# thu-ml/zhusuan

Measured on NVIDIA H100. Metric: leapfrog-steps*chains/sec, higher is better.
Workload: dtype f32

## Files before the change

zhusuan_b200/csrc/hmc_dense_res.cu:

```cuda
#include "hmc_dense_epilogue.cuh"

namespace {

struct ResEpi {
  const __half* __restrict__ hi_cur; const __half* __restrict__ lo_cur;
  __half* __restrict__ hi_nxt; __half* __restrict__ lo_nxt;
  const __half* __restrict__ hi_cur_s; const __half* __restrict__ lo_cur_s;
  __half* __restrict__ hi_nxt_s; __half* __restrict__ lo_nxt_s;
  const float* __restrict__ p_in; float* __restrict__ p_out;
  float* __restrict__ lp_part; float* __restrict__ k_part;
  int64_t chains; int D;
  float sq, inv_sq, acc_scale;
  float rescale;
};

template <int MODE, int NEXT, int DC, bool SPARE>
__device__ __forceinline__ void epilogue_planes(const ResEpi& a, uint32_t trow, int n, bool n_ok,
                                                int64_t c0, int64_t part_row, int lane, float s2,
                                                float eps_over_m_sq, float inv_m, float b_n,
                                                float mu_n, float& qmax) {
  constexpr int NCOL = BN;
  const uint32_t D = DC ? (uint32_t)DC : (uint32_t)a.D;
  const int64_t chains = a.chains;
  const bool warp_n_ok = __all_sync(0xffffffffu, n_ok);
  const bool fast_tile = warp_n_ok && (c0 + NCOL <= chains);
  const int64_t off_t = c0 * (int64_t)D + n;
  const float* __restrict__ pin0 = a.p_in + off_t;
  float* __restrict__ po0 = a.p_out + off_t;
  const unsigned short* __restrict__ hc0 =
      reinterpret_cast<const unsigned short*>(a.hi_cur) + off_t;
  const unsigned short* __restrict__ lc0 =
      reinterpret_cast<const unsigned short*>(a.lo_cur) + off_t;
  __half* __restrict__ hn0 = NEXT ? a.hi_nxt + off_t : nullptr;
  __half* __restrict__ ln0 = NEXT ? a.lo_nxt + off_t : nullptr;
  __half* __restrict__ hs0 = SPARE ? a.hi_nxt_s + off_t : nullptr;
  __half* __restrict__ ls0 = SPARE ? a.lo_nxt_s + off_t : nullptr;

  auto element = [&](float acc, float p, uint32_t hl, float& pn, float& lpv, float& kv,
                     float& Qn) {
    const float Q = __half2float(__ushort_as_half((unsigned short)(hl & 0xFFFFu))) +
                    __half2float(__ushort_as_half((unsigned short)(hl >> 16)));
    const float g = b_n - a.acc_scale * acc;
    pn = fmaf(s2, g, p);
    if (MODE >= 1) lpv = (Q * a.inv_sq - mu_n) * g;
    if (MODE >= 2) kv = pn * pn * inv_m;
    if (NEXT) Qn = fmaf(eps_over_m_sq, pn, Q);
  };

  if (fast_tile) {
    auto load = [&](float* pe, uint32_t* he, int c) {
      const size_t cb = (size_t)c * D;
#pragma unroll
      for (int j = 0; j < 16; ++j) {
        pe[j] = __ldcg(pin0 + cb + (uint32_t)j * D);
        const uint32_t h = __ldcg(hc0 + cb + (uint32_t)j * D);
        const uint32_t l = __ldcg(lc0 + cb + (uint32_t)j * D);
        he[j] = h | (l << 16);
      }
    };
    float ss_a = 0.f, ss_b = 0.f;
    auto compute = [&](const uint32_t* v, const float* pe, const uint32_t* he, int c, float& ss) {
      const size_t cb = (size_t)c * D;
      float lpv[MODE >= 1 ? 16 : 1], kv[MODE >= 2 ? 16 : 1];
#pragma unroll
      for (int j = 0; j < 16; j += 2) {
        float pn[2], lp1[2] = {0.f, 0.f}, k1[2] = {0.f, 0.f}, Qn[2] = {0.f, 0.f};
#pragma unroll
        for (int t = 0; t < 2; ++t) {
          element(__uint_as_float(v[j + t]), pe[j + t], he[j + t], pn[t], lp1[t], k1[t], Qn[t]);
          po0[cb + (uint32_t)(j + t) * D] = pn[t];
          if (MODE >= 1) lpv[j + t] = lp1[t];
          if (MODE >= 2) kv[j + t] = k1[t];
          if (NEXT && !SPARE) ss = fmaf(Qn[t], Qn[t], ss);
          if (SPARE) qmax = fmaxf(qmax, fabsf(Qn[t]));
        }
        if (NEXT) {
          const __half2 h2 = __floats2half2_rn(Qn[0], Qn[1]);
          const float2 hf = __half22float2(h2);
          const __half2 l2 = __floats2half2_rn(Qn[0] - hf.x, Qn[1] - hf.y);
          hn0[cb + (uint32_t)j * D] = __low2half(h2);
          hn0[cb + (uint32_t)(j + 1) * D] = __high2half(h2);
          ln0[cb + (uint32_t)j * D] = __low2half(l2);
          ln0[cb + (uint32_t)(j + 1) * D] = __high2half(l2);
        }
        if (SPARE) {
          const float x0 = Qn[0] * a.rescale, x1 = Qn[1] * a.rescale;
          const __half2 h2 = __floats2half2_rn(x0, x1);
          const float2 hf = __half22float2(h2);
          const __half2 l2 = __floats2half2_rn(x0 - hf.x, x1 - hf.y);
          hs0[cb + (uint32_t)j * D] = __low2half(h2);
          hs0[cb + (uint32_t)(j + 1) * D] = __high2half(h2);
          ls0[cb + (uint32_t)j * D] = __low2half(l2);
          ls0[cb + (uint32_t)(j + 1) * D] = __high2half(l2);
        }
      }
      if (MODE >= 1) {
        const float sum = warp_transpose_sum16(lpv, lane);
        if (lane < 16) a.lp_part[part_row + c0 + c + lane] = sum;
      }
      if (MODE >= 2) {
        const float sum = warp_transpose_sum16(kv, lane);
        if (lane < 16) a.k_part[part_row + c0 + c + lane] = sum;
      }
    };
    float pa[16], pb[16];
    uint32_t ha[16], hb[16], va[16], vb[16];
    load(pa, ha, 0);
#pragma unroll 1
    for (int c = 0; c < NCOL; c += 32) {
      load(pb, hb, c + 16);
      acc_ld16(trow + 4u * (uint32_t)c, va);
      compute(va, pa, ha, c, ss_a);
      if (c + 32 < NCOL) load(pa, ha, c + 32);
      acc_ld16(trow + 4u * (uint32_t)(c + 16), vb);
      compute(vb, pb, hb, c + 16, ss_b);
    }
    if (NEXT && !SPARE) {
      const float norm = sqrtf(ss_a + ss_b) * (1.f + 0x1p-10f);
      qmax = fmaxf(qmax, norm == norm ? norm : INFINITY);
    }
  } else {
#pragma unroll 1
    for (int c = 0; c < NCOL; c += 16) {
      uint32_t v[16];
      acc_ld16(trow + 4u * (uint32_t)c, v);
      const int64_t cbase = c0 + c;
      if (cbase < chains) {
        const size_t cb = (size_t)c * D;
        float lpv[MODE >= 1 ? 16 : 1], kv[MODE >= 2 ? 16 : 1];
#pragma unroll
        for (int j = 0; j < 16; ++j) {
          const bool ok = n_ok && cbase + j < chains;
          float p = 0.f;
          uint32_t hl = 0u;
          if (ok) {
            p = __ldcg(pin0 + cb + (uint32_t)j * D);
            hl = (uint32_t)__ldcg(hc0 + cb + (uint32_t)j * D) |
                 ((uint32_t)__ldcg(lc0 + cb + (uint32_t)j * D) << 16);
          }
          float pn, lp1 = 0.f, k1 = 0.f, Qn = 0.f;
          element(__uint_as_float(v[j]), p, hl, pn, lp1, k1, Qn);
          const __half hh = __float2half_rn(Qn);
          const __half ll = __float2half_rn(Qn - __half2float(hh));
          if (NEXT && ok) qmax = fmaxf(qmax, fabsf(Qn));
          if (MODE >= 1) lpv[j] = ok ? lp1 : 0.f;
          if (MODE >= 2) kv[j] = ok ? k1 : 0.f;
          if (ok) {
            po0[cb + (uint32_t)j * D] = pn;
            if (NEXT) {
              hn0[cb + (uint32_t)j * D] = hh;
              ln0[cb + (uint32_t)j * D] = ll;
            }
            if (SPARE) {
              const float x = Qn * a.rescale;
              const __half hs = __float2half_rn(x);
              hs0[cb + (uint32_t)j * D] = hs;
              ls0[cb + (uint32_t)j * D] = __float2half_rn(x - __half2float(hs));
            }
          }
        }
        if (MODE >= 1) {
          const float sum = warp_transpose_sum16(lpv, lane);
          if (lane < 16 && cbase + lane < chains) a.lp_part[part_row + cbase + lane] = sum;
        }
        if (MODE >= 2) {
          const float sum = warp_transpose_sum16(kv, lane);
          if (lane < 16 && cbase + lane < chains) a.k_part[part_row + cbase + lane] = sum;
        }
      }
    }
  }
}


__device__ __forceinline__ int& producer_spare_in() {
  __shared__ int spare_in;
  return spare_in;
}

template <int MODE, int NEXT, int DC, int CX, int CY>
struct ResW {
  static constexpr int KIND = 1, RB = 64, MNA = 0, MNB = 0;
  static constexpr int CLUSTER = CX * CY;
  static constexpr int KE = RB / 2;
  static constexpr uint32_t TX = Cfg<RB>::STAGE;
  CUtensorMap m_phi, m_plo, m_qhi, m_qlo, m_shi, m_slo;
  ResEpi ea;
  const float* bvec; const float* mu; const float* mass; const float* state;
  float* scales;
  float p_scale;
  int n_blk, D_rt, pass;
  struct EpiState { float qmax = 0.f; };

  __device__ __forceinline__ int D() const { return DC ? DC : D_rt; }
  __host__ __device__ __forceinline__ int64_t units() const {
    return ((ea.chains + BN - 1) / BN) * (int64_t)n_blk;
  }
  __device__ __forceinline__ void tile(int64_t u, int& nb, int64_t& cb) const {
    const uint64_t cu = (uint64_t)u / CLUSTER;
    const int r = (int)((uint64_t)u % CLUSTER);
    const uint32_t nbx = (uint32_t)(n_blk / CX);
    nb = (int)(cu % nbx) * CX + r % CX;
    cb = (int64_t)(cu / nbx) * CY + r / CX;
  }
  __device__ __forceinline__ void kb_range(int64_t, int& kb0, int& kb1) const {
    kb0 = 0;
    kb1 = D() / KE;
  }
  __device__ __forceinline__ void prefetch() const {
    tma_prefetch_desc(&m_phi); tma_prefetch_desc(&m_plo);
    tma_prefetch_desc(&m_qhi); tma_prefetch_desc(&m_qlo);
    tma_prefetch_desc(&m_shi); tma_prefetch_desc(&m_slo);
    producer_spare_in() = plane_spare_in(scales, pass);
  }
  __device__ __forceinline__ void load(int64_t u, int kb, uint32_t sa, uint32_t fb) const {
    using C = Cfg<RB>;
    int nb;
    int64_t cb;
    tile(u, nb, cb);
    const int n0 = nb * BM;
    const int c0 = (int)cb * BN;
    const bool s = producer_spare_in() != 0;
    const CUtensorMap* qh = s ? &m_shi : &m_qhi;
    const CUtensorMap* ql = s ? &m_slo : &m_qlo;
    const int r = (int)(u % CLUSTER), rx = r % CX, ry = r / CX;
    if constexpr (CY == 1) {
      tma_load_2d(sa, &m_phi, fb, kb * KE, n0);
      tma_load_2d(sa + C::A_TILE, &m_plo, fb, kb * KE, n0);
    } else {
      constexpr int rows = BM / CY;
      uint16_t mask = 0;
#pragma unroll
      for (int y = 0; y < CY; ++y) mask |= (uint16_t)(1u << (y * CX + rx));
      const uint32_t o = (uint32_t)(ry * rows * RB);
      tma_load_2d_mc(sa + o, &m_phi, fb, kb * KE, n0 + ry * rows, mask);
      tma_load_2d_mc(sa + C::A_TILE + o, &m_plo, fb, kb * KE, n0 + ry * rows, mask);
    }
    if constexpr (CX == 1) {
      tma_load_2d(sa + 2 * C::A_TILE, qh, fb, kb * KE, c0);
      tma_load_2d(sa + 2 * C::A_TILE + C::B_TILE, ql, fb, kb * KE, c0);
    } else {
      constexpr int rows = BN / CX;
      const uint16_t mask = (uint16_t)(((1u << CX) - 1u) << (ry * CX));
      const uint32_t o = (uint32_t)(rx * rows * RB);
      tma_load_2d_mc(sa + 2 * C::A_TILE + o, qh, fb, kb * KE, c0 + rx * rows, mask);
      tma_load_2d_mc(sa + 2 * C::A_TILE + C::B_TILE + o, ql, fb, kb * KE, c0 + rx * rows, mask);
    }
  }
  __device__ __forceinline__ float sq_alt(float eps, float sq) const {
    return next_plane_scale(scales, pass, eps, mul(eps, p_scale), sq);
  }
  __device__ __forceinline__ void epilogue(int64_t u, uint32_t trow, int quarter, int lane,
                                           EpiState& st) const {
    int nb;
    int64_t cb;
    tile(u, nb, cb);
    const int n = nb * BM + quarter * 32 + lane;
    const int64_t c0 = cb * BN;
    const bool n_ok = n < D();
    const float eps = state[ZSB_ST_EPS_USED];
    const float s2 = mul(eps, p_scale);
    const bool spare_in = plane_spare_in(scales, pass);
    const float sq = plane_scale_in(scales, pass);
    const float m_n = n_ok ? mass[n] : 1.f;
    const float eps_over_m_sq = mul(fdiv(eps, m_n), sq);
    const float inv_m = fdiv(1.f, m_n);
    const float b_n = (n_ok && bvec) ? bvec[n] : 0.f;
    const float mu_n = (n_ok && mu) ? mu[n] : 0.f;
    const int64_t part_row = (int64_t)(nb * 4 + quarter) * ea.chains;
    ResEpi a = ea;
    if (spare_in) {
      a.hi_cur = ea.hi_cur_s;
      a.lo_cur = ea.lo_cur_s;
    }
    a.sq = sq;
    a.inv_sq = fdiv(1.f, sq);
    a.acc_scale = 1.f / (scales[3] * sq);
    a.rescale = NEXT ? sq_alt(eps, sq) * a.inv_sq : 1.f;
    if (a.rescale == 1.f)
      epilogue_planes<MODE, NEXT, DC, false>(a, trow, n, n_ok, c0, part_row, lane, s2,
                                             eps_over_m_sq, inv_m, b_n, mu_n, st.qmax);
    else
      epilogue_planes<MODE, NEXT, DC, true>(a, trow, n, n_ok, c0, part_row, lane, s2,
                                            eps_over_m_sq, inv_m, b_n, mu_n, st.qmax);
  }
  __device__ __forceinline__ void epi_finish(EpiState& st, int quarter, int lane) const {
    if (!NEXT) return;
    const float sq = plane_scale_in(scales, pass);
    const float alt = sq_alt(state[ZSB_ST_EPS_USED], sq);
    publish_plane_scale(scales, pass, sq, alt, st.qmax * (1.f / sq),
                        alt != sq && !(st.qmax < kHalfOverflow), quarter, lane);
  }
};

constexpr int RES_CX = 2, RES_CY = 1;

template <int DC, int CX, int CY>
int res_pass(const CUtensorMap& phi, const CUtensorMap& plo, const CUtensorMap& qhi,
             const CUtensorMap& qlo, const CUtensorMap& shi, const CUtensorMap& slo,
             const ResEpi& ea, const float* bvec, const float* mu, const float* mass,
             const float* state, float* scales, int pass, float p_scale, int n_blk, int D,
             int mode, cudaStream_t st) {
  if (mode == 1) {
    const ResW<1, 1, DC, CX, CY> w{phi, plo, qhi, qlo, shi, slo, ea, bvec, mu, mass, state,
                                   scales, p_scale, n_blk, D, pass};
    return tc_launch(w, st, "hmc_dense_resident");
  }
  if (mode == 0) {
    const ResW<0, 1, DC, CX, CY> w{phi, plo, qhi, qlo, shi, slo, ea, bvec, mu, mass, state,
                                   scales, p_scale, n_blk, D, pass};
    return tc_launch(w, st, "hmc_dense_resident");
  }
  const ResW<2, 0, DC, CX, CY> w{phi, plo, qhi, qlo, shi, slo, ea, bvec, mu, mass, state, scales,
                                 p_scale, n_blk, D, pass};
  return tc_launch(w, st, "hmc_dense_resident");
}

template <int DC>
int res_pass(bool cluster, const CUtensorMap& phi, const CUtensorMap& plo, const CUtensorMap& qhi,
             const CUtensorMap& qlo, const CUtensorMap& shi, const CUtensorMap& slo,
             const ResEpi& ea, const float* bvec, const float* mu, const float* mass,
             const float* state, float* scales, int pass, float p_scale, int n_blk, int D,
             int mode, cudaStream_t st) {
  return cluster ? res_pass<DC, RES_CX, RES_CY>(phi, plo, qhi, qlo, shi, slo, ea, bvec, mu, mass,
                                                state, scales, pass, p_scale, n_blk, D, mode, st)
                 : res_pass<DC, 1, 1>(phi, plo, qhi, qlo, shi, slo, ea, bvec, mu, mass, state,
                                      scales, pass, p_scale, n_blk, D, mode, st);
}

__global__ void __launch_bounds__(256) select_planes_kernel(float* __restrict__ q,
                                                            const __half* __restrict__ planes,
                                                            const __half* __restrict__ spare,
                                                            const float* __restrict__ record,
                                                            const int32_t* __restrict__ accept,
                                                            int64_t chains, int64_t D) {
  const bool use_spare = __float_as_uint(record[3]) != 0u;
  const float inv_sq = 1.f / record[use_spare ? 1 : 0];
  if (use_spare) planes = spare;
  const int lane = threadIdx.x & 31;
  const int n8 = (int)(D >> 3);
  const int64_t wstride = (int64_t)gridDim.x * 8;
  for (int64_t c = (int64_t)blockIdx.x * 8 + (threadIdx.x >> 5); c < chains; c += wstride) {
    if (!accept[c]) continue;
    const uint4* __restrict__ hi = reinterpret_cast<const uint4*>(planes + c * D);
    const uint4* __restrict__ lo = reinterpret_cast<const uint4*>(planes + (chains + c) * D);
    float4* __restrict__ qr = reinterpret_cast<float4*>(q + c * D);
    for (int i0 = lane; i0 < n8; i0 += 128) {
      uint4 h[4], l[4];
#pragma unroll
      for (int u = 0; u < 4; ++u) {
        const int i = i0 + 32 * u;
        if (i < n8) { h[u] = __ldcs(hi + i); l[u] = __ldcs(lo + i); }
      }
#pragma unroll
      for (int u = 0; u < 4; ++u) {
        const int i = i0 + 32 * u;
        if (i < n8) {
          const uint32_t hw[4] = {h[u].x, h[u].y, h[u].z, h[u].w};
          const uint32_t lw[4] = {l[u].x, l[u].y, l[u].z, l[u].w};
          float o[8];
#pragma unroll
          for (int k = 0; k < 4; ++k) {
            const float2 hf = __half22float2(*reinterpret_cast<const __half2*>(&hw[k]));
            const float2 lf = __half22float2(*reinterpret_cast<const __half2*>(&lw[k]));
            o[2 * k] = (hf.x + lf.x) * inv_sq;
            o[2 * k + 1] = (hf.y + lf.y) * inv_sq;
          }
          qr[2 * i] = make_float4(o[0], o[1], o[2], o[3]);
          qr[2 * i + 1] = make_float4(o[4], o[5], o[6], o[7]);
        }
      }
    }
  }
}

}

int zsb_dense_res_h16_launch(void* planes0, void* planes1, void* spare0, void* spare1,
                             const float* p0, float* pw,
                             const void* P_h16, const void* P_l16, float* scales,
                             const float* bvec, const float* mu, const float* mass,
                             const float* state, float* lp0_part, float* lp1_part, float* k_part,
                             int64_t chains, int D, int L, cudaStream_t st) {
  if (D % 64 != 0 || D < 64 || L < 1 || chains <= 0 || chains >= (1LL << 31)) {
    zsb_set_error("dense_res: needs D %% 64 == 0, n_leapfrogs >= 1");
    return ZSB_ERR_INVALID;
  }
  if (planes0 == planes1 || !spare0 || !spare1 || spare0 == spare1) {
    zsb_set_error("dense_res: planes1, spare0 and spare1 must be separate work buffers");
    return ZSB_ERR_INVALID;
  }
  const int n_blk = (D + BM - 1) / BM;
  const int64_t c_blk = (chains + BN - 1) / BN;
  const bool cluster = n_blk % RES_CX == 0 && c_blk % RES_CY == 0;
  const uint32_t p_box = cluster ? BM / RES_CY : BM, q_box = cluster ? BN / RES_CX : BN;
  CUtensorMap phi, plo, qhi[2], qlo[2], shi[2], slo[2];
  int rc;
  constexpr int RB = ResW<0, 1, 0, 1, 1>::RB;
  if ((rc = make_map(&phi, P_h16, (uint64_t)D, (uint64_t)D, p_box, RB, 1))) return rc;
  if ((rc = make_map(&plo, P_l16, (uint64_t)D, (uint64_t)D, p_box, RB, 1))) return rc;
  __half* pl[2] = {reinterpret_cast<__half*>(planes0), reinterpret_cast<__half*>(planes1)};
  __half* sp[2] = {reinterpret_cast<__half*>(spare0), reinterpret_cast<__half*>(spare1)};
  const int64_t plane = chains * (int64_t)D;
  for (int b = 0; b < 2; ++b) {
    if ((rc = make_map(&qhi[b], pl[b], (uint64_t)chains, (uint64_t)D, q_box, RB, 1))) return rc;
    if ((rc = make_map(&qlo[b], pl[b] + plane, (uint64_t)chains, (uint64_t)D, q_box, RB, 1)))
      return rc;
    if ((rc = make_map(&shi[b], sp[b], (uint64_t)chains, (uint64_t)D, q_box, RB, 1))) return rc;
    if ((rc = make_map(&slo[b], sp[b] + plane, (uint64_t)chains, (uint64_t)D, q_box, RB, 1)))
      return rc;
  }
  for (int i = 0; i <= L; ++i) {
    const bool last = i == L;
    const int buf = i & 1;
    const ResEpi ea{pl[buf], pl[buf] + plane, pl[buf ^ 1], pl[buf ^ 1] + plane,
                    sp[buf], sp[buf] + plane, sp[buf ^ 1], sp[buf ^ 1] + plane,
                    i == 0 ? p0 : pw, pw, i == 0 ? lp0_part : lp1_part, k_part, chains, D,
                    1.f, 1.f, 1.f, 1.f};
    const int mode = last ? 2 : (i == 0 ? 1 : 0);
    const float p_scale = (i > 0 && !last) ? 1.f : 0.5f;
    rc = (D == 1024)
             ? res_pass<1024>(cluster, phi, plo, qhi[buf], qlo[buf], shi[buf], slo[buf], ea, bvec,
                              mu, mass, state, scales, i, p_scale, n_blk, D, mode, st)
             : res_pass<0>(cluster, phi, plo, qhi[buf], qlo[buf], shi[buf], slo[buf], ea, bvec, mu,
                           mass, state, scales, i, p_scale, n_blk, D, mode, st);
    if (rc != ZSB_OK) return rc;
  }
  return ZSB_OK;
}

#ifdef ZSB_PASS_PROFILE
extern "C" int zsb_pass_profile_read(unsigned long long* host, int ctas) {
  if (ctas < 0 || ctas > PASS_PROF_CTAS) return ZSB_ERR_INVALID;
  const size_t bytes = sizeof(unsigned long long) * PASS_PROF_SLOTS * (size_t)ctas;
  if (cudaMemcpyFromSymbol(host, g_pass_prof, bytes) != cudaSuccess) return ZSB_ERR_CUDA;
  static unsigned long long zeros[PASS_PROF_CTAS * PASS_PROF_SLOTS];
  if (cudaMemcpyToSymbol(g_pass_prof, zeros, sizeof(zeros)) != cudaSuccess) return ZSB_ERR_CUDA;
  return ZSB_OK;
}
#endif

int zsb_dense_select_planes_launch(float* q, const void* planes, const void* spare,
                                   const float* record, const int32_t* accept, int64_t chains,
                                   int64_t D, cudaStream_t st) {
  ZSB_REQUIRE(D % 8 == 0, "zsb_dense_select_planes: D must be a multiple of 8");
  int64_t blocks = zsb_ceil_div(chains, 8);
  if (blocks > ZSB_NUM_SMS * 16) blocks = ZSB_NUM_SMS * 16;
  if (blocks < 1) blocks = 1;
  select_planes_kernel<<<(unsigned)blocks, 256, 0, st>>>(
      q, reinterpret_cast<const __half*>(planes), reinterpret_cast<const __half*>(spare), record,
      accept, chains, D);
  return zsb_check_launch("hmc_select_planes");
}
```

zhusuan_b200/csrc/tc_common.cuh:

```cuda
#pragma once
#include "common.cuh"
#include <cuda.h>
#include <cuda_fp16.h>

namespace {

constexpr int BM = 128;
constexpr int BN = 128;
constexpr int NUM_EPI_WARPS = 4;
constexpr int PRODUCER_WARP = 4;
constexpr int EPI_WARP0 = 5;
constexpr int NUM_THREADS = 32 * (EPI_WARP0 + NUM_EPI_WARPS);
constexpr int ACC_LD = BN + 4;
constexpr int ACC_BYTES = BM * ACC_LD * 4;
constexpr unsigned long long WAIT_TIMEOUT_NS = 2000000000ULL;

enum PassProfSlot {
  PROF_MMA_TOTAL,
  PROF_MMA_FULL,
  PROF_MMA_TEMPTY,
  PROF_MMA_STORE,
  PROF_PROD_EMPTY,
  PROF_EPI_TFULL,
  PROF_EPI_UNIT,
  PROF_UNITS,
  PASS_PROF_SLOTS
};
constexpr int PASS_PROF_CTAS = 1024;
#ifdef ZSB_PASS_PROFILE
constexpr bool kPassProfile = true;
__device__ unsigned long long g_pass_prof[PASS_PROF_CTAS * PASS_PROF_SLOTS];
#else
constexpr bool kPassProfile = false;
#endif
__device__ __forceinline__ long long prof_clock() {
  if constexpr (kPassProfile) return clock64();
  return 0;
}
__device__ __forceinline__ void prof_add(int slot, long long v) {
#ifdef ZSB_PASS_PROFILE
  if (blockIdx.x < PASS_PROF_CTAS)
    atomicAdd(&g_pass_prof[blockIdx.x * PASS_PROF_SLOTS + slot], (unsigned long long)v);
#endif
}

template <int RB>
struct Cfg {
  static constexpr int A_TILE = BM * RB;
  static constexpr int B_TILE = BN * RB;
  static constexpr int STAGE = 2 * A_TILE + 2 * B_TILE;
  static constexpr int STAGES = RB == 128 ? 2 : 5;
  static constexpr int ALIGN = RB == 128 ? 1024 : 512;
  static constexpr int SMEM = STAGES * STAGE + ACC_BYTES + 128 + ALIGN;
  static_assert(SMEM <= 227 * 1024, "operand ring exceeds shared memory");
};

__device__ __forceinline__ uint32_t smem_u32(const void* p) {
  return (uint32_t)__cvta_generic_to_shared(p);
}
__device__ __forceinline__ void mbar_init(uint32_t bar, uint32_t count) {
  asm volatile("mbarrier.init.shared::cta.b64 [%0], %1;" ::"r"(bar), "r"(count) : "memory");
}
__device__ __forceinline__ void mbar_expect_tx(uint32_t bar, uint32_t bytes) {
  asm volatile("mbarrier.arrive.expect_tx.shared::cta.b64 _, [%0], %1;" ::"r"(bar), "r"(bytes)
               : "memory");
}
__device__ __forceinline__ void mbar_arrive(uint32_t bar) {
  asm volatile("mbarrier.arrive.shared::cta.b64 _, [%0];" ::"r"(bar) : "memory");
}
__device__ __forceinline__ bool mbar_try_wait(uint32_t bar, uint32_t parity) {
  uint32_t ok;
  asm volatile(
      "{\n\t.reg .pred P1;\n\t"
      "mbarrier.try_wait.parity.shared::cta.b64 P1, [%1], %2;\n\t"
      "selp.b32 %0, 1, 0, P1;\n\t}"
      : "=r"(ok)
      : "r"(bar), "r"(parity)
      : "memory");
  return ok != 0;
}
__device__ __forceinline__ unsigned long long global_ns() {
  unsigned long long t;
  asm volatile("mov.u64 %0, %%globaltimer;" : "=l"(t));
  return t;
}
__device__ __forceinline__ void mbar_wait(uint32_t bar, uint32_t parity) {
  if (mbar_try_wait(bar, parity)) return;
  const unsigned long long t0 = global_ns();
  while (!mbar_try_wait(bar, parity))
    if (global_ns() - t0 > WAIT_TIMEOUT_NS) __trap();
}
__device__ __forceinline__ void mbar_spin(uint32_t bar, uint32_t parity) {
  while (!mbar_try_wait(bar, parity)) {
  }
}
__device__ __forceinline__ void tma_load_2d(uint32_t dst, const CUtensorMap* map, uint32_t bar,
                                            int c0, int c1) {
  asm volatile(
      "cp.async.bulk.tensor.2d.shared::cluster.global.mbarrier::complete_tx::bytes"
      " [%0], [%1, {%3, %4}], [%2];"
      ::"r"(dst), "l"(map), "r"(bar), "r"(c0), "r"(c1)
      : "memory");
}
__device__ __forceinline__ void tma_load_2d_mc(uint32_t dst, const CUtensorMap* map, uint32_t bar,
                                               int c0, int c1, uint16_t mask) {
  asm volatile(
      "cp.async.bulk.tensor.2d.shared::cluster.global.mbarrier::complete_tx::bytes"
      ".multicast::cluster [%0], [%1, {%3, %4}], [%2], %5;"
      ::"r"(dst), "l"(map), "r"(bar), "r"(c0), "r"(c1), "h"(mask)
      : "memory");
}
__device__ __forceinline__ void mbar_arrive_cluster(uint32_t bar, uint32_t cta) {
  asm volatile(
      "{\n\t.reg .b32 rb;\n\t"
      "mapa.shared::cluster.u32 rb, %0, %1;\n\t"
      "mbarrier.arrive.shared::cluster.b64 _, [rb];\n\t}"
      ::"r"(bar), "r"(cta)
      : "memory");
}
__device__ __forceinline__ void cluster_sync() {
  asm volatile("barrier.cluster.arrive.release;\n\tbarrier.cluster.wait.acquire;" ::: "memory");
}
__device__ __forceinline__ void tma_prefetch_desc(const CUtensorMap* map) {
  asm volatile("prefetch.tensormap [%0];" ::"l"(map) : "memory");
}

template <int MN, int RB>
__device__ __forceinline__ uint64_t gmma_desc(uint32_t saddr) {
  uint64_t d = (uint64_t)((saddr & 0x3FFFF) >> 4);
  if (MN) {
    d |= (uint64_t)(8192 >> 4) << 16;
    d |= (uint64_t)(1024 >> 4) << 32;
    d |= (uint64_t)1 << 62;
  } else {
    d |= (uint64_t)1 << 16;
    d |= (uint64_t)((8 * RB) >> 4) << 32;
    d |= (uint64_t)(RB == 128 ? 1 : 2) << 62;
  }
  return d;
}
__device__ __forceinline__ void wgmma_fence() {
  asm volatile("wgmma.fence.sync.aligned;" ::: "memory");
}
__device__ __forceinline__ void wgmma_commit() {
  asm volatile("wgmma.commit_group.sync.aligned;" ::: "memory");
}
template <int N>
__device__ __forceinline__ void wgmma_wait() {
  asm volatile("wgmma.wait_group.sync.aligned %0;" ::"n"(N) : "memory");
}
__device__ __forceinline__ void wgmma_tf32(float (&d)[64], uint64_t da, uint64_t db) {
  asm volatile(
      "{\n\t.reg .pred p;\n\tsetp.ne.b32 p, 1, 0;\n\t"
      "wgmma.mma_async.sync.aligned.m64n128k8.f32.tf32.tf32 {%0, %1, %2, %3, %4, %5, %6, %7, %8, %9, %10, %11, %12, %13, %14, %15, %16, %17, %18, %19, %20, %21, %22, %23, %24, %25, %26, %27, %28, %29, %30, %31, %32, %33, %34, %35, %36, %37, %38, %39, %40, %41, %42, %43, %44, %45, %46, %47, %48, %49, %50, %51, %52, %53, %54, %55, %56, %57, %58, %59, %60, %61, %62, %63}, %64, %65, p, 1, 1;\n\t}"
      : "+f"(d[0]), "+f"(d[1]), "+f"(d[2]), "+f"(d[3]), "+f"(d[4]), "+f"(d[5]), "+f"(d[6]), "+f"(d[7]), "+f"(d[8]), "+f"(d[9]), "+f"(d[10]), "+f"(d[11]), "+f"(d[12]), "+f"(d[13]), "+f"(d[14]), "+f"(d[15]), "+f"(d[16]), "+f"(d[17]), "+f"(d[18]), "+f"(d[19]), "+f"(d[20]), "+f"(d[21]), "+f"(d[22]), "+f"(d[23]), "+f"(d[24]), "+f"(d[25]), "+f"(d[26]), "+f"(d[27]), "+f"(d[28]), "+f"(d[29]), "+f"(d[30]), "+f"(d[31]), "+f"(d[32]), "+f"(d[33]), "+f"(d[34]), "+f"(d[35]), "+f"(d[36]), "+f"(d[37]), "+f"(d[38]), "+f"(d[39]), "+f"(d[40]), "+f"(d[41]), "+f"(d[42]), "+f"(d[43]), "+f"(d[44]), "+f"(d[45]), "+f"(d[46]), "+f"(d[47]), "+f"(d[48]), "+f"(d[49]), "+f"(d[50]), "+f"(d[51]), "+f"(d[52]), "+f"(d[53]), "+f"(d[54]), "+f"(d[55]), "+f"(d[56]), "+f"(d[57]), "+f"(d[58]), "+f"(d[59]), "+f"(d[60]), "+f"(d[61]), "+f"(d[62]), "+f"(d[63])
      : "l"(da), "l"(db));
}
template <int TA, int TB>
__device__ __forceinline__ void wgmma_f16(float (&d)[64], uint64_t da, uint64_t db) {
  asm volatile(
      "{\n\t.reg .pred p;\n\tsetp.ne.b32 p, 1, 0;\n\t"
      "wgmma.mma_async.sync.aligned.m64n128k16.f32.f16.f16 {%0, %1, %2, %3, %4, %5, %6, %7, %8, %9, %10, %11, %12, %13, %14, %15, %16, %17, %18, %19, %20, %21, %22, %23, %24, %25, %26, %27, %28, %29, %30, %31, %32, %33, %34, %35, %36, %37, %38, %39, %40, %41, %42, %43, %44, %45, %46, %47, %48, %49, %50, %51, %52, %53, %54, %55, %56, %57, %58, %59, %60, %61, %62, %63}, %64, %65, p, 1, 1, %66, %67;\n\t}"
      : "+f"(d[0]), "+f"(d[1]), "+f"(d[2]), "+f"(d[3]), "+f"(d[4]), "+f"(d[5]), "+f"(d[6]), "+f"(d[7]), "+f"(d[8]), "+f"(d[9]), "+f"(d[10]), "+f"(d[11]), "+f"(d[12]), "+f"(d[13]), "+f"(d[14]), "+f"(d[15]), "+f"(d[16]), "+f"(d[17]), "+f"(d[18]), "+f"(d[19]), "+f"(d[20]), "+f"(d[21]), "+f"(d[22]), "+f"(d[23]), "+f"(d[24]), "+f"(d[25]), "+f"(d[26]), "+f"(d[27]), "+f"(d[28]), "+f"(d[29]), "+f"(d[30]), "+f"(d[31]), "+f"(d[32]), "+f"(d[33]), "+f"(d[34]), "+f"(d[35]), "+f"(d[36]), "+f"(d[37]), "+f"(d[38]), "+f"(d[39]), "+f"(d[40]), "+f"(d[41]), "+f"(d[42]), "+f"(d[43]), "+f"(d[44]), "+f"(d[45]), "+f"(d[46]), "+f"(d[47]), "+f"(d[48]), "+f"(d[49]), "+f"(d[50]), "+f"(d[51]), "+f"(d[52]), "+f"(d[53]), "+f"(d[54]), "+f"(d[55]), "+f"(d[56]), "+f"(d[57]), "+f"(d[58]), "+f"(d[59]), "+f"(d[60]), "+f"(d[61]), "+f"(d[62]), "+f"(d[63])
      : "l"(da), "l"(db), "n"(TA), "n"(TB));
}

__device__ __forceinline__ void acc_ld16(uint32_t addr, uint32_t v[16]) {
#pragma unroll
  for (int i = 0; i < 4; ++i)
    asm volatile("ld.shared.v4.b32 {%0, %1, %2, %3}, [%4];"
                 : "=r"(v[4 * i]), "=r"(v[4 * i + 1]), "=r"(v[4 * i + 2]), "=r"(v[4 * i + 3])
                 : "r"(addr + 16u * i));
}

__device__ __forceinline__ float warp_transpose_sum16(float v[16], int lane) {
#pragma unroll
  for (int i = 0; i < 16; ++i) v[i] += __shfl_xor_sync(0xffffffffu, v[i], 16);
#pragma unroll
  for (int o = 8, cnt = 16; o >= 1; o >>= 1, cnt >>= 1) {
    const bool upper = (lane & o) != 0;
#pragma unroll
    for (int i = 0; i < cnt / 2; ++i) {
      const float keep = upper ? v[i + cnt / 2] : v[i];
      const float send = upper ? v[i] : v[i + cnt / 2];
      v[i] = keep + __shfl_xor_sync(0xffffffffu, send, o);
    }
  }
  return v[0];
}

__device__ __forceinline__ float pow2_plane_scale(float m) {
  int e = 0;
  if (m > 0.f) frexpf(m, &e);
  return ldexpf(1.f, 12 - e);
}
__device__ __forceinline__ float finite_absmax(float m, float x) {
  const float a = fabsf(x);
  return (a <= 3.0e38f) ? fmaxf(m, a) : m;
}
__device__ __forceinline__ void store_hilo(__half* p, int64_t lo, float x) {
  const __half h = __float2half_rn(x);
  p[0] = h;
  p[lo] = __float2half_rn(x - __half2float(h));
}
__device__ __forceinline__ void fold_amax(float* scale, float m, int lane) {
  m = warp_max(m);
  if (lane == 0 && m > 0.f) atomicMax(reinterpret_cast<unsigned int*>(scale) + 2, __float_as_uint(m));
}

template <int KIND, int RB, int MNA, int MNB, int ZLO = 0>
__device__ __forceinline__ void mma_kblock(float (&d)[2][64], uint32_t sa) {
  using C = Cfg<RB>;
#pragma unroll
  for (int k = 0; k < RB / 32; ++k) {
    const uint32_t bo = MNB ? (uint32_t)k * 2048u : (uint32_t)k * 32u;
    const uint64_t b_hi = gmma_desc<MNB, RB>(sa + 2 * C::A_TILE + bo);
    const uint64_t b_lo = gmma_desc<MNB, RB>(sa + 2 * C::A_TILE + C::B_TILE + bo);
#pragma unroll
    for (int mh = 0; mh < 2; ++mh) {
      const uint32_t ao = MNA ? (uint32_t)mh * 8192u + (uint32_t)k * 2048u
                              : (uint32_t)(mh * 64 * RB) + (uint32_t)k * 32u;
      const uint64_t a_hi = gmma_desc<MNA, RB>(sa + ao);
      const uint64_t a_lo = gmma_desc<MNA, RB>(sa + C::A_TILE + ao);
      if (KIND == 0) {
        wgmma_tf32(d[mh], a_lo, b_hi);
        wgmma_tf32(d[mh], a_hi, b_lo);
        wgmma_tf32(d[mh], a_hi, b_hi);
      } else {
        if (!(ZLO & 1)) wgmma_f16<MNA, MNB>(d[mh], a_lo, b_hi);
        if (!(ZLO & 2)) wgmma_f16<MNA, MNB>(d[mh], a_hi, b_lo);
        wgmma_f16<MNA, MNB>(d[mh], a_hi, b_hi);
      }
    }
  }
}

template <class W, class = void>
struct ClusterOf {
  static constexpr int value = 1;
};
template <class W>
struct ClusterOf<W, decltype((void)W::CLUSTER)> {
  static constexpr int value = W::CLUSTER;
};

template <class W, class = void>
struct ZloOf {
  static constexpr int value = 0;
};
template <class W>
struct ZloOf<W, decltype((void)W::ZLO)> {
  static constexpr int value = W::ZLO;
};

template <class W>
__global__ void __launch_bounds__(NUM_THREADS, 1) tc_pipeline_kernel(const __grid_constant__ W w) {
  using C = Cfg<W::RB>;
  constexpr int CS = ClusterOf<W>::value;
  extern __shared__ uint8_t smem_raw[];
  const uint32_t smem_base = (smem_u32(smem_raw) + (C::ALIGN - 1)) & ~(uint32_t)(C::ALIGN - 1);
  const uint32_t acc_base = smem_base + C::STAGES * C::STAGE;
  const uint32_t bars = acc_base + ACC_BYTES;
  const uint32_t full_bar = bars;
  const uint32_t empty_bar = bars + 8 * C::STAGES;
  const uint32_t tfull_bar = bars + 16 * C::STAGES;
  const uint32_t tempty_bar = tfull_bar + 8;

  const int warp = __shfl_sync(0xffffffffu, (int)(threadIdx.x >> 5), 0);
  const int lane = threadIdx.x & 31;
  const int64_t n_units = w.units();

  if (threadIdx.x == 0) {
    for (int s = 0; s < C::STAGES; ++s) {
      mbar_init(full_bar + 8 * s, 1);
      mbar_init(empty_bar + 8 * s, CS);
    }
    mbar_init(tfull_bar, 128);
    mbar_init(tempty_bar, 32 * NUM_EPI_WARPS);
    asm volatile("fence.mbarrier_init.release.cluster;" ::: "memory");
  }
  if constexpr (CS > 1)
    cluster_sync();
  else
    __syncthreads();
  auto release = [&](int s) {
    if constexpr (CS > 1) {
#pragma unroll
      for (int r = 0; r < CS; ++r) mbar_arrive_cluster(empty_bar + 8 * s, (uint32_t)r);
    } else {
      mbar_arrive(empty_bar + 8 * s);
    }
  };

  if (warp < 4) {
    const int tid = threadIdx.x;
    float d[2][64];
    int stage = 0;
    uint32_t phase = 0, acc_phase = 0;
    const long long t_begin = prof_clock();
    long long t_full = 0, t_tempty = 0, t_store = 0, units = 0;
    for (int64_t u = blockIdx.x; u < n_units; u += gridDim.x) {
      int kb0, kb1;
      w.kb_range(u, kb0, kb1);
#pragma unroll
      for (int mh = 0; mh < 2; ++mh)
#pragma unroll
        for (int i = 0; i < 64; ++i) d[mh][i] = 0.f;
      int prev = -1;
      for (int kb = kb0; kb < kb1; ++kb) {
        const uint32_t sa = smem_base + stage * C::STAGE;
        const long long t0 = prof_clock();
        mbar_spin(full_bar + 8 * stage, phase);
        t_full += prof_clock() - t0;
        wgmma_fence();
        mma_kblock<W::KIND, W::RB, W::MNA, W::MNB, ZloOf<W>::value>(d, sa);
        wgmma_commit();
        wgmma_wait<1>();
        if (prev >= 0 && tid == 0) release(prev);
        prev = stage;
        if (++stage == C::STAGES) { stage = 0; phase ^= 1; }
      }
      wgmma_wait<0>();
      if (prev >= 0 && tid == 0) release(prev);
      const long long t1 = prof_clock();
      mbar_wait(tempty_bar, acc_phase ^ 1);
      const long long t2 = prof_clock();
      t_tempty += t2 - t1;
      const int row = 16 * (tid >> 5) + ((tid & 31) >> 2);
      const int col = 2 * (tid & 3);
#pragma unroll
      for (int mh = 0; mh < 2; ++mh)
#pragma unroll
        for (int j = 0; j < 16; ++j) {
          const uint32_t a0 = acc_base + (uint32_t)(((64 * mh + row) * ACC_LD + 8 * j + col) * 4);
          asm volatile("st.shared.v2.f32 [%0], {%1, %2};" ::"r"(a0), "f"(d[mh][4 * j]),
                       "f"(d[mh][4 * j + 1]) : "memory");
          asm volatile("st.shared.v2.f32 [%0], {%1, %2};" ::"r"(a0 + 8u * ACC_LD * 4u),
                       "f"(d[mh][4 * j + 2]), "f"(d[mh][4 * j + 3]) : "memory");
        }
      mbar_arrive(tfull_bar);
      acc_phase ^= 1;
      t_store += prof_clock() - t2;
      ++units;
    }
    if (kPassProfile && tid == 0) {
      prof_add(PROF_MMA_TOTAL, prof_clock() - t_begin);
      prof_add(PROF_MMA_FULL, t_full);
      prof_add(PROF_MMA_TEMPTY, t_tempty);
      prof_add(PROF_MMA_STORE, t_store);
      prof_add(PROF_UNITS, units);
    }
  } else if (warp == PRODUCER_WARP) {
    if (lane == 0) {
      w.prefetch();
      int stage = 0;
      uint32_t phase = 0;
      long long t_empty = 0;
      for (int64_t u = blockIdx.x; u < n_units; u += gridDim.x) {
        int kb0, kb1;
        w.kb_range(u, kb0, kb1);
        for (int kb = kb0; kb < kb1; ++kb) {
          const long long t0 = prof_clock();
          mbar_wait(empty_bar + 8 * stage, phase ^ 1);
          t_empty += prof_clock() - t0;
          const uint32_t fb = full_bar + 8 * stage;
          mbar_expect_tx(fb, W::TX);
          w.load(u, kb, smem_base + stage * C::STAGE, fb);
          if (++stage == C::STAGES) { stage = 0; phase ^= 1; }
        }
      }
      if (kPassProfile) prof_add(PROF_PROD_EMPTY, t_empty);
    }
  } else {
    const int quarter = warp - EPI_WARP0;
    const uint32_t trow = acc_base + (uint32_t)((quarter * 32 + lane) * ACC_LD * 4);
    typename W::EpiState st;
    uint32_t acc_phase = 0;
    long long t_tfull = 0, t_unit = 0;
    for (int64_t u = blockIdx.x; u < n_units; u += gridDim.x) {
      const long long t0 = prof_clock();
      mbar_wait(tfull_bar, acc_phase);
      const long long t1 = prof_clock();
      w.epilogue(u, trow, quarter, lane, st);
      __syncwarp();
      mbar_arrive(tempty_bar);
      acc_phase ^= 1;
      t_tfull += t1 - t0;
      t_unit += prof_clock() - t1;
    }
    if (kPassProfile && quarter == 0 && lane == 0) {
      prof_add(PROF_EPI_TFULL, t_tfull);
      prof_add(PROF_EPI_UNIT, t_unit);
    }
    w.epi_finish(st, quarter, lane);
  }
  if constexpr (CS > 1) cluster_sync();
}

template <class W>
int tc_launch(const W& w, cudaStream_t st, const char* what) {
  constexpr int CS = ClusterOf<W>::value;
  static const cudaError_t attr = cudaFuncSetAttribute(
      tc_pipeline_kernel<W>, cudaFuncAttributeMaxDynamicSharedMemorySize, Cfg<W::RB>::SMEM);
  if (attr != cudaSuccess) {
    zsb_set_error("%s: cudaFuncSetAttribute: %s", what, cudaGetErrorString(attr));
    return ZSB_ERR_CUDA;
  }
  if constexpr (CS > 1) {
    const int64_t units = w.units();
    if (units < 1 || units % CS != 0) {
      zsb_set_error("%s: %lld units do not tile by clusters of %d", what, (long long)units, CS);
      return ZSB_ERR_INVALID;
    }
    cudaLaunchAttribute cl[1];
    cl[0].id = cudaLaunchAttributeClusterDimension;
    cl[0].val.clusterDim.x = CS;
    cl[0].val.clusterDim.y = 1;
    cl[0].val.clusterDim.z = 1;
    cudaLaunchConfig_t cfg = {};
    cfg.blockDim = dim3(NUM_THREADS);
    cfg.dynamicSmemBytes = Cfg<W::RB>::SMEM;
    cfg.stream = st;
    cfg.attrs = cl;
    cfg.numAttrs = 1;
    static int max_clusters = 0;
    if (max_clusters < 1) {
      cfg.gridDim = dim3(CS);
      const cudaError_t e =
          cudaOccupancyMaxActiveClusters(&max_clusters, tc_pipeline_kernel<W>, &cfg);
      if (e != cudaSuccess || max_clusters < 1) {
        zsb_set_error("%s: no cluster of %d CTAs fits (%s)", what, CS, cudaGetErrorString(e));
        max_clusters = 0;
        return ZSB_ERR_CUDA;
      }
    }
    int64_t grid = (int64_t)max_clusters * CS;
    if (grid > units) grid = units;
    cfg.gridDim = dim3((unsigned)grid);
    const cudaError_t e = cudaLaunchKernelEx(&cfg, tc_pipeline_kernel<W>, w);
    if (e != cudaSuccess) {
      zsb_set_error("%s: cudaLaunchKernelEx: %s", what, cudaGetErrorString(e));
      return ZSB_ERR_CUDA;
    }
    return zsb_check_launch(what);
  } else {
    int dev = 0, sms = ZSB_NUM_SMS;
    cudaGetDevice(&dev);
    cudaDeviceGetAttribute(&sms, cudaDevAttrMultiProcessorCount, dev);
    int64_t grid = w.units();
    if (grid > sms) grid = sms;
    if (grid < 1) grid = 1;
    tc_pipeline_kernel<W><<<(unsigned)grid, NUM_THREADS, Cfg<W::RB>::SMEM, st>>>(w);
    return zsb_check_launch(what);
  }
}

typedef CUresult (*EncodeTiledFn)(CUtensorMap*, CUtensorMapDataType, cuuint32_t, void*,
                                  const cuuint64_t*, const cuuint64_t*, const cuuint32_t*,
                                  const cuuint32_t*, CUtensorMapInterleave, CUtensorMapSwizzle,
                                  CUtensorMapL2promotion, CUtensorMapFloatOOBfill);

EncodeTiledFn get_encode_fn() {
  static EncodeTiledFn fn = nullptr;
  if (!fn) {
    void* p = nullptr;
    cudaDriverEntryPointQueryResult qres;
    if (cudaGetDriverEntryPoint("cuTensorMapEncodeTiled", &p, cudaEnableDefault, &qres) !=
            cudaSuccess || qres != cudaDriverEntryPointSuccess)
      return nullptr;
    fn = (EncodeTiledFn)p;
  }
  return fn;
}

int make_map(CUtensorMap* map, const void* base, uint64_t rows, uint64_t cols, uint32_t box_rows,
             int rb, int half_elems = 0) {
  EncodeTiledFn enc = get_encode_fn();
  if (!enc) {
    zsb_set_error("tc: cuTensorMapEncodeTiled unavailable");
    return ZSB_ERR_CUDA;
  }
  const int esz = half_elems ? 2 : 4;
  cuuint64_t dims[2] = {cols, rows};
  cuuint64_t strides[1] = {cols * esz};
  cuuint32_t box[2] = {(cuuint32_t)(rb / esz), box_rows};
  cuuint32_t estr[2] = {1, 1};
  CUresult r = enc(map, half_elems ? CU_TENSOR_MAP_DATA_TYPE_FLOAT16 : CU_TENSOR_MAP_DATA_TYPE_FLOAT32,
                   2, (void*)base, dims, strides, box, estr,
                   CU_TENSOR_MAP_INTERLEAVE_NONE,
                   rb == 128 ? CU_TENSOR_MAP_SWIZZLE_128B : CU_TENSOR_MAP_SWIZZLE_64B,
                   CU_TENSOR_MAP_L2_PROMOTION_L2_256B, CU_TENSOR_MAP_FLOAT_OOB_FILL_NONE);
  if (r != CUDA_SUCCESS) {
    zsb_set_error("tc: cuTensorMapEncodeTiled failed (%d)", (int)r);
    return ZSB_ERR_CUDA;
  }
  return ZSB_OK;
}

}
```

Before: 72.80 million.

## Widen residual GEMM tile to 160 chains with register reallocation

```diff
diff --git a/zhusuan_b200/csrc/hmc_dense_res.cu b/zhusuan_b200/csrc/hmc_dense_res.cu
--- a/zhusuan_b200/csrc/hmc_dense_res.cu
+++ b/zhusuan_b200/csrc/hmc_dense_res.cu
@@ -14,12 +14,12 @@
   float rescale;
 };
 
-template <int MODE, int NEXT, int DC, bool SPARE>
+template <int MODE, int NEXT, int DC, bool SPARE, int NCOL>
 __device__ __forceinline__ void epilogue_planes(const ResEpi& a, uint32_t trow, int n, bool n_ok,
                                                 int64_t c0, int64_t part_row, int lane, float s2,
                                                 float eps_over_m_sq, float inv_m, float b_n,
                                                 float mu_n, float& qmax) {
-  constexpr int NCOL = BN;
+  constexpr int NORM_COLS = NCOL > 128 ? 96 : 128;
   const uint32_t D = DC ? (uint32_t)DC : (uint32_t)a.D;
   const int64_t chains = a.chains;
   const bool warp_n_ok = __all_sync(0xffffffffu, n_ok);
@@ -103,6 +103,11 @@
         if (lane < 16) a.k_part[part_row + c0 + c + lane] = sum;
       }
     };
+    auto fold_norm = [&]() {
+      const float norm = sqrtf(ss_a + ss_b) * (1.f + 0x1p-10f);
+      qmax = fmaxf(qmax, norm == norm ? norm : INFINITY);
+      ss_a = ss_b = 0.f;
+    };
     float pa[16], pb[16];
     uint32_t ha[16], hb[16], va[16], vb[16];
     load(pa, ha, 0);
@@ -114,11 +119,9 @@
       if (c + 32 < NCOL) load(pa, ha, c + 32);
       acc_ld16(trow + 4u * (uint32_t)(c + 16), vb);
       compute(vb, pb, hb, c + 16, ss_b);
-    }
-    if (NEXT && !SPARE) {
-      const float norm = sqrtf(ss_a + ss_b) * (1.f + 0x1p-10f);
-      qmax = fmaxf(qmax, norm == norm ? norm : INFINITY);
-    }
+      if (NEXT && !SPARE && NCOL > NORM_COLS && c + 32 == NORM_COLS) fold_norm();
+    }
+    if (NEXT && !SPARE) fold_norm();
   } else {
 #pragma unroll 1
     for (int c = 0; c < NCOL; c += 16) {
@@ -178,12 +181,14 @@
   return spare_in;
 }
 
+constexpr int RES_BN = 160;
+
 template <int MODE, int NEXT, int DC, int CX, int CY>
 struct ResW {
-  static constexpr int KIND = 1, RB = 64, MNA = 0, MNB = 0;
+  static constexpr int KIND = 1, RB = 64, MNA = 0, MNB = 0, BN = RES_BN;
   static constexpr int CLUSTER = CX * CY;
   static constexpr int KE = RB / 2;
-  static constexpr uint32_t TX = Cfg<RB>::STAGE;
+  static constexpr uint32_t TX = Cfg<RB, BN>::STAGE;
   CUtensorMap m_phi, m_plo, m_qhi, m_qlo, m_shi, m_slo;
   ResEpi ea;
   const float* bvec; const float* mu; const float* mass; const float* state;
@@ -214,7 +219,7 @@
     producer_spare_in() = plane_spare_in(scales, pass);
   }
   __device__ __forceinline__ void load(int64_t u, int kb, uint32_t sa, uint32_t fb) const {
-    using C = Cfg<RB>;
+    using C = Cfg<RB, BN>;
     int nb;
     int64_t cb;
     tile(u, nb, cb);
@@ -278,11 +283,11 @@
     a.acc_scale = 1.f / (scales[3] * sq);
     a.rescale = NEXT ? sq_alt(eps, sq) * a.inv_sq : 1.f;
     if (a.rescale == 1.f)
-      epilogue_planes<MODE, NEXT, DC, false>(a, trow, n, n_ok, c0, part_row, lane, s2,
-                                             eps_over_m_sq, inv_m, b_n, mu_n, st.qmax);
+      epilogue_planes<MODE, NEXT, DC, false, BN>(a, trow, n, n_ok, c0, part_row, lane, s2,
+                                                 eps_over_m_sq, inv_m, b_n, mu_n, st.qmax);
     else
-      epilogue_planes<MODE, NEXT, DC, true>(a, trow, n, n_ok, c0, part_row, lane, s2,
-                                            eps_over_m_sq, inv_m, b_n, mu_n, st.qmax);
+      epilogue_planes<MODE, NEXT, DC, true, BN>(a, trow, n, n_ok, c0, part_row, lane, s2,
+                                                eps_over_m_sq, inv_m, b_n, mu_n, st.qmax);
   }
   __device__ __forceinline__ void epi_finish(EpiState& st, int quarter, int lane) const {
     if (!NEXT) return;
@@ -391,9 +396,10 @@
     return ZSB_ERR_INVALID;
   }
   const int n_blk = (D + BM - 1) / BM;
-  const int64_t c_blk = (chains + BN - 1) / BN;
+  const int64_t c_blk = (chains + RES_BN - 1) / RES_BN;
   const bool cluster = n_blk % RES_CX == 0 && c_blk % RES_CY == 0;
-  const uint32_t p_box = cluster ? BM / RES_CY : BM, q_box = cluster ? BN / RES_CX : BN;
+  const uint32_t p_box = cluster ? BM / RES_CY : BM;
+  const uint32_t q_box = cluster ? RES_BN / RES_CX : RES_BN;
   CUtensorMap phi, plo, qhi[2], qlo[2], shi[2], slo[2];
   int rc;
   constexpr int RB = ResW<0, 1, 0, 1, 1>::RB;
diff --git a/zhusuan_b200/csrc/tc_common.cuh b/zhusuan_b200/csrc/tc_common.cuh
--- a/zhusuan_b200/csrc/tc_common.cuh
+++ b/zhusuan_b200/csrc/tc_common.cuh
@@ -9,10 +9,6 @@
 constexpr int BN = 128;
 constexpr int NUM_EPI_WARPS = 4;
 constexpr int PRODUCER_WARP = 4;
-constexpr int EPI_WARP0 = 5;
-constexpr int NUM_THREADS = 32 * (EPI_WARP0 + NUM_EPI_WARPS);
-constexpr int ACC_LD = BN + 4;
-constexpr int ACC_BYTES = BM * ACC_LD * 4;
 constexpr unsigned long long WAIT_TIMEOUT_NS = 2000000000ULL;
 
 enum PassProfSlot {
@@ -44,15 +40,21 @@
 #endif
 }
 
-template <int RB>
+template <int RB, int N_ = BN>
 struct Cfg {
+  static constexpr int N = N_;
+  static constexpr bool WIDE = N > 128;
+  static constexpr int EPI_WARP0 = WIDE ? 8 : 5;
+  static constexpr int THREADS = 32 * (EPI_WARP0 + NUM_EPI_WARPS);
+  static constexpr int ACC_LD = N + 4;
+  static constexpr int ACC_BYTES = BM * ACC_LD * 4;
   static constexpr int A_TILE = BM * RB;
-  static constexpr int B_TILE = BN * RB;
+  static constexpr int B_TILE = N * RB;
   static constexpr int STAGE = 2 * A_TILE + 2 * B_TILE;
-  static constexpr int STAGES = RB == 128 ? 2 : 5;
   static constexpr int ALIGN = RB == 128 ? 1024 : 512;
+  static constexpr int STAGES = (227 * 1024 - ACC_BYTES - 128 - ALIGN) / STAGE;
   static constexpr int SMEM = STAGES * STAGE + ACC_BYTES + 128 + ALIGN;
-  static_assert(SMEM <= 227 * 1024, "operand ring exceeds shared memory");
+  static_assert(N % 32 == 0 && STAGES >= 2, "unit too wide for the operand ring");
 };
 
 __device__ __forceinline__ uint32_t smem_u32(const void* p) {
@@ -165,6 +167,15 @@
       : "l"(da), "l"(db), "n"(TA), "n"(TB));
 }
 
+template <int TA, int TB>
+__device__ __forceinline__ void wgmma_f16(float (&d)[80], uint64_t da, uint64_t db) {
+  asm volatile(
+      "{\n\t.reg .pred p;\n\tsetp.ne.b32 p, 1, 0;\n\t"
+      "wgmma.mma_async.sync.aligned.m64n160k16.f32.f16.f16 {%0, %1, %2, %3, %4, %5, %6, %7, %8, %9, %10, %11, %12, %13, %14, %15, %16, %17, %18, %19, %20, %21, %22, %23, %24, %25, %26, %27, %28, %29, %30, %31, %32, %33, %34, %35, %36, %37, %38, %39, %40, %41, %42, %43, %44, %45, %46, %47, %48, %49, %50, %51, %52, %53, %54, %55, %56, %57, %58, %59, %60, %61, %62, %63, %64, %65, %66, %67, %68, %69, %70, %71, %72, %73, %74, %75, %76, %77, %78, %79}, %80, %81, p, 1, 1, %82, %83;\n\t}"
+      : "+f"(d[0]), "+f"(d[1]), "+f"(d[2]), "+f"(d[3]), "+f"(d[4]), "+f"(d[5]), "+f"(d[6]), "+f"(d[7]), "+f"(d[8]), "+f"(d[9]), "+f"(d[10]), "+f"(d[11]), "+f"(d[12]), "+f"(d[13]), "+f"(d[14]), "+f"(d[15]), "+f"(d[16]), "+f"(d[17]), "+f"(d[18]), "+f"(d[19]), "+f"(d[20]), "+f"(d[21]), "+f"(d[22]), "+f"(d[23]), "+f"(d[24]), "+f"(d[25]), "+f"(d[26]), "+f"(d[27]), "+f"(d[28]), "+f"(d[29]), "+f"(d[30]), "+f"(d[31]), "+f"(d[32]), "+f"(d[33]), "+f"(d[34]), "+f"(d[35]), "+f"(d[36]), "+f"(d[37]), "+f"(d[38]), "+f"(d[39]), "+f"(d[40]), "+f"(d[41]), "+f"(d[42]), "+f"(d[43]), "+f"(d[44]), "+f"(d[45]), "+f"(d[46]), "+f"(d[47]), "+f"(d[48]), "+f"(d[49]), "+f"(d[50]), "+f"(d[51]), "+f"(d[52]), "+f"(d[53]), "+f"(d[54]), "+f"(d[55]), "+f"(d[56]), "+f"(d[57]), "+f"(d[58]), "+f"(d[59]), "+f"(d[60]), "+f"(d[61]), "+f"(d[62]), "+f"(d[63]), "+f"(d[64]), "+f"(d[65]), "+f"(d[66]), "+f"(d[67]), "+f"(d[68]), "+f"(d[69]), "+f"(d[70]), "+f"(d[71]), "+f"(d[72]), "+f"(d[73]), "+f"(d[74]), "+f"(d[75]), "+f"(d[76]), "+f"(d[77]), "+f"(d[78]), "+f"(d[79])
+      : "l"(da), "l"(db), "n"(TA), "n"(TB));
+}
+
 __device__ __forceinline__ void acc_ld16(uint32_t addr, uint32_t v[16]) {
 #pragma unroll
   for (int i = 0; i < 4; ++i)
@@ -208,9 +219,10 @@
   if (lane == 0 && m > 0.f) atomicMax(reinterpret_cast<unsigned int*>(scale) + 2, __float_as_uint(m));
 }
 
-template <int KIND, int RB, int MNA, int MNB, int ZLO = 0>
-__device__ __forceinline__ void mma_kblock(float (&d)[2][64], uint32_t sa) {
-  using C = Cfg<RB>;
+template <int KIND, int RB, int MNA, int MNB, int ZLO = 0, int N = BN>
+__device__ __forceinline__ void mma_kblock(float (&d)[2][N / 2], uint32_t sa) {
+  using C = Cfg<RB, N>;
+  static_assert(N == 128 || (KIND == 1 && MNB == 0), "wide units: fp16, K-major B only");
 #pragma unroll
   for (int k = 0; k < RB / 32; ++k) {
     const uint32_t bo = MNB ? (uint32_t)k * 2048u : (uint32_t)k * 32u;
@@ -222,7 +234,7 @@
                               : (uint32_t)(mh * 64 * RB) + (uint32_t)k * 32u;
       const uint64_t a_hi = gmma_desc<MNA, RB>(sa + ao);
       const uint64_t a_lo = gmma_desc<MNA, RB>(sa + C::A_TILE + ao);
-      if (KIND == 0) {
+      if constexpr (KIND == 0) {
         wgmma_tf32(d[mh], a_lo, b_hi);
         wgmma_tf32(d[mh], a_hi, b_lo);
         wgmma_tf32(d[mh], a_hi, b_hi);
@@ -253,14 +265,38 @@
   static constexpr int value = W::ZLO;
 };
 
+template <class W, class = void>
+struct BnOf {
+  static constexpr int value = BN;
+};
 template <class W>
-__global__ void __launch_bounds__(NUM_THREADS, 1) tc_pipeline_kernel(const __grid_constant__ W w) {
-  using C = Cfg<W::RB>;
+struct BnOf<W, decltype((void)W::BN)> {
+  static constexpr int value = W::BN;
+};
+template <class W>
+using CfgOf = Cfg<W::RB, BnOf<W>::value>;
+
+constexpr int WIDE_MMA_REGS = 232, WIDE_PRODUCER_REGS = 40, WIDE_EPI_REGS = 232;
+static_assert(WIDE_MMA_REGS + WIDE_PRODUCER_REGS + WIDE_EPI_REGS <= 3 * (65536 / 384 / 8 * 8),
+              "wide layout: register budgets exceed the launch allocation");
+template <int R>
+__device__ __forceinline__ void setmaxnreg_inc() {
+  asm volatile("setmaxnreg.inc.sync.aligned.u32 %0;" ::"n"(R));
+}
+template <int R>
+__device__ __forceinline__ void setmaxnreg_dec() {
+  asm volatile("setmaxnreg.dec.sync.aligned.u32 %0;" ::"n"(R));
+}
+
+template <class W>
+__global__ void __launch_bounds__(CfgOf<W>::THREADS, 1)
+    tc_pipeline_kernel(const __grid_constant__ W w) {
+  using C = CfgOf<W>;
   constexpr int CS = ClusterOf<W>::value;
   extern __shared__ uint8_t smem_raw[];
   const uint32_t smem_base = (smem_u32(smem_raw) + (C::ALIGN - 1)) & ~(uint32_t)(C::ALIGN - 1);
   const uint32_t acc_base = smem_base + C::STAGES * C::STAGE;
-  const uint32_t bars = acc_base + ACC_BYTES;
+  const uint32_t bars = acc_base + C::ACC_BYTES;
   const uint32_t full_bar = bars;
   const uint32_t empty_bar = bars + 8 * C::STAGES;
   const uint32_t tfull_bar = bars + 16 * C::STAGES;
@@ -293,8 +329,9 @@
   };
 
   if (warp < 4) {
+    if constexpr (C::WIDE) setmaxnreg_inc<WIDE_MMA_REGS>();
     const int tid = threadIdx.x;
-    float d[2][64];
+    float d[2][C::N / 2];
     int stage = 0;
     uint32_t phase = 0, acc_phase = 0;
     const long long t_begin = prof_clock();
@@ -305,7 +342,7 @@
 #pragma unroll
       for (int mh = 0; mh < 2; ++mh)
 #pragma unroll
-        for (int i = 0; i < 64; ++i) d[mh][i] = 0.f;
+        for (int i = 0; i < C::N / 2; ++i) d[mh][i] = 0.f;
       int prev = -1;
       for (int kb = kb0; kb < kb1; ++kb) {
         const uint32_t sa = smem_base + stage * C::STAGE;
@@ -313,7 +350,7 @@
         mbar_spin(full_bar + 8 * stage, phase);
         t_full += prof_clock() - t0;
         wgmma_fence();
-        mma_kblock<W::KIND, W::RB, W::MNA, W::MNB, ZloOf<W>::value>(d, sa);
+        mma_kblock<W::KIND, W::RB, W::MNA, W::MNB, ZloOf<W>::value, C::N>(d, sa);
         wgmma_commit();
         wgmma_wait<1>();
         if (prev >= 0 && tid == 0) release(prev);
@@ -331,11 +368,11 @@
 #pragma unroll
       for (int mh = 0; mh < 2; ++mh)
 #pragma unroll
-        for (int j = 0; j < 16; ++j) {
-          const uint32_t a0 = acc_base + (uint32_t)(((64 * mh + row) * ACC_LD + 8 * j + col) * 4);
+        for (int j = 0; j < C::N / 8; ++j) {
+          const uint32_t a0 = acc_base + (uint32_t)(((64 * mh + row) * C::ACC_LD + 8 * j + col) * 4);
           asm volatile("st.shared.v2.f32 [%0], {%1, %2};" ::"r"(a0), "f"(d[mh][4 * j]),
                        "f"(d[mh][4 * j + 1]) : "memory");
-          asm volatile("st.shared.v2.f32 [%0], {%1, %2};" ::"r"(a0 + 8u * ACC_LD * 4u),
+          asm volatile("st.shared.v2.f32 [%0], {%1, %2};" ::"r"(a0 + 8u * C::ACC_LD * 4u),
                        "f"(d[mh][4 * j + 2]), "f"(d[mh][4 * j + 3]) : "memory");
         }
       mbar_arrive(tfull_bar);
@@ -350,8 +387,9 @@
       prof_add(PROF_MMA_STORE, t_store);
       prof_add(PROF_UNITS, units);
     }
-  } else if (warp == PRODUCER_WARP) {
-    if (lane == 0) {
+  } else if (warp < C::EPI_WARP0) {
+    if constexpr (C::WIDE) setmaxnreg_dec<WIDE_PRODUCER_REGS>();
+    if (warp == PRODUCER_WARP && lane == 0) {
       w.prefetch();
       int stage = 0;
       uint32_t phase = 0;
@@ -372,8 +410,9 @@
       if (kPassProfile) prof_add(PROF_PROD_EMPTY, t_empty);
     }
   } else {
-    const int quarter = warp - EPI_WARP0;
-    const uint32_t trow = acc_base + (uint32_t)((quarter * 32 + lane) * ACC_LD * 4);
+    if constexpr (C::WIDE) setmaxnreg_inc<WIDE_EPI_REGS>();
+    const int quarter = warp - C::EPI_WARP0;
+    const uint32_t trow = acc_base + (uint32_t)((quarter * 32 + lane) * C::ACC_LD * 4);
     typename W::EpiState st;
     uint32_t acc_phase = 0;
     long long t_tfull = 0, t_unit = 0;
@@ -400,8 +439,9 @@
 template <class W>
 int tc_launch(const W& w, cudaStream_t st, const char* what) {
   constexpr int CS = ClusterOf<W>::value;
+  using C = CfgOf<W>;
   static const cudaError_t attr = cudaFuncSetAttribute(
-      tc_pipeline_kernel<W>, cudaFuncAttributeMaxDynamicSharedMemorySize, Cfg<W::RB>::SMEM);
+      tc_pipeline_kernel<W>, cudaFuncAttributeMaxDynamicSharedMemorySize, C::SMEM);
   if (attr != cudaSuccess) {
     zsb_set_error("%s: cudaFuncSetAttribute: %s", what, cudaGetErrorString(attr));
     return ZSB_ERR_CUDA;
@@ -418,8 +458,8 @@
     cl[0].val.clusterDim.y = 1;
     cl[0].val.clusterDim.z = 1;
     cudaLaunchConfig_t cfg = {};
-    cfg.blockDim = dim3(NUM_THREADS);
-    cfg.dynamicSmemBytes = Cfg<W::RB>::SMEM;
+    cfg.blockDim = dim3(C::THREADS);
+    cfg.dynamicSmemBytes = C::SMEM;
     cfg.stream = st;
     cfg.attrs = cl;
     cfg.numAttrs = 1;
@@ -450,7 +490,7 @@
     int64_t grid = w.units();
     if (grid > sms) grid = sms;
     if (grid < 1) grid = 1;
-    tc_pipeline_kernel<W><<<(unsigned)grid, NUM_THREADS, Cfg<W::RB>::SMEM, st>>>(w);
+    tc_pipeline_kernel<W><<<(unsigned)grid, C::THREADS, C::SMEM, st>>>(w);
     return zsb_check_launch(what);
   }
 }
```

Result: faster. 74.94 million (median of 6 runs) (+2.9%).
